# AlerianEmperor/Voxel-Cone-Tracing

Hardware: AMD Instinct MI355X
Metric: Mcones/s (+ ms per GI pass), Sponza-class 256^3 @1080p (higher is better)
Workload: dtype f32; 1 GPU; procedural atrium (Sponza-class, 257488 tris, seed 1234), 256^3 RGBA8 brick chain, 1920x1080, 6 diffuse + 1 specular cone/px, trace of a resident (GPU-rasterised) G-buffer; voxel_dim=256, width=1920, height=1080, cones_per_pixel=7, bounces=1, anisotropic_mips=False, parallelism=single GPU, trace_variant=0, footprint_records=False, comm_reserved_cus=0, raster_form=direct

## Files before the change

### voxel-cone-tracing_amd/csrc/vct_trace.hip

```cpp
#include <hip/hip_fp16.h>

#include "../../include/vct.h"
#include "vct_internal.h"

typedef int vct_v4i32 __attribute__((ext_vector_type(4)));
typedef float vct_v4f32 __attribute__((ext_vector_type(4)));
__device__ vct_v4f32 vct_struct_buffer_load_format_v4f32(vct_v4i32 rsrc, int vindex, int voffset, int soffset, int aux)
    __asm("llvm.amdgcn.struct.buffer.load.format.v4f32");

namespace {

struct F3 { float x, y, z; };
struct F4 { float x, y, z, w; };

__device__ __forceinline__ F3 f3(float x, float y, float z) { return {x, y, z}; }
__device__ __forceinline__ float dot3(F3 a, F3 b) { return a.x * b.x + a.y * b.y + a.z * b.z; }
__device__ __forceinline__ F3 cross3(F3 a, F3 b) {
    return {a.y * b.z - a.z * b.y, a.z * b.x - a.x * b.z, a.x * b.y - a.y * b.x};
}
__device__ __forceinline__ float div_rn(float a, float b) { return a / b; }
__device__ __forceinline__ float sqrt_rn(float a) { return __builtin_sqrtf(a); }
__device__ __forceinline__ F3 normalize3(F3 a) {
    const float l = sqrt_rn(dot3(a, a));
    return {div_rn(a.x, l), div_rn(a.y, l), div_rn(a.z, l)};
// ... 100 lines not shown
        ay = __builtin_amdgcn_readlane(j0, src) - 1;
        az = __builtin_amdgcn_readlane(k0, src) - 1;
        dx = i0 - ax; dy = j0 - ay; dz = k0 - az;
        const uint32_t far = max(max((uint32_t)dx, (uint32_t)dy), (uint32_t)dz);
        const unsigned long long out = ballot64(far > 2u) & am;
        coop = out == 0ull;
    }
    if (COOP && coop) {
        uint32_t idx;
        if (WRAP) {
            const uint32_t m4 = (uint32_t)m << 2;
            const uint32_t sax = spread_byte(lb.lut, ax, m4) >> 2;
            const uint32_t say = spread_byte(lb.lut, ay, m4) >> 1;
            const uint32_t saz = spread_byte(lb.lut, az, m4);
            idx = (((sax | ~MX) + lb.sbx) & MX) | (((say | ~MY) + lb.sby) & MY) |
                  (((saz | ~MZ) + lb.sbz) & MZ);
        } else {
            const int x = min(max(ax + (lb.lane & 3), 0), m);
            const int y = min(max(ay + ((lb.lane >> 2) & 3), 0), m);
            const int z = min(max(az + (lb.lane >> 4), 0), m);
            idx = vct_morton3((uint32_t)x, (uint32_t)y, (uint32_t)z);
        }
        const float4 d = texel_f32(tb, idx);
        if (PRIO) __builtin_amdgcn_s_setprio(0);
        const bool any_texel = ballot64((__float_as_uint(d.x) | __float_as_uint(d.y) | __float_as_uint(d.z) | __float_as_uint(d.w)) != 0u) != 0ull;
        if (VCT_STATS) { if (any_texel) ++ms.coop_hit; else ++ms.coop_zero; }
        if (any_texel) {
            blk[lb.lane] = d;
            wave_sync();
            const int slot = act ? (dz * 4 + dy) * 4 + dx : 0;
            const float4* q = blk + slot;
            const float a0 = 1.0f - a, b0 = 1.0f - b, c0 = 1.0f - c;
            const float ab00 = a0 * b0, ab10 = a * b0, ab01 = a0 * b, ab11 = a * b;
            {
                const float4 t0 = q[0], t1 = q[1], t2 = q[4], t3 = q[5];
                const float w0 = ab00 * c0, w1 = ab10 * c0, w2 = ab01 * c0, w3 = ab11 * c0;
#define VCT_ACC(ch) r.ch = w0 * t0.ch; r.ch = fmaf(w1, t1.ch, r.ch); r.ch = fmaf(w2, t2.ch, r.ch); r.ch = fmaf(w3, t3.ch, r.ch);
                VCT_ACC(x) VCT_ACC(y) VCT_ACC(z) VCT_ACC(w)
#undef VCT_ACC
            }
            __builtin_amdgcn_sched_barrier(0);
            {
                const float4 t4 = q[16], t5 = q[17], t6 = q[20], t7 = q[21];
                wave_sync();
                const float w4 = ab00 * c, w5 = ab10 * c, w6 = ab01 * c, w7 = ab11 * c;
#define VCT_ACC(ch) r.ch = fmaf(w4, t4.ch, r.ch); r.ch = fmaf(w5, t5.ch, r.ch); r.ch = fmaf(w6, t6.ch, r.ch); r.ch = fmaf(w7, t7.ch, r.ch);
                VCT_ACC(x) VCT_ACC(y) VCT_ACC(z) VCT_ACC(w)
#undef VCT_ACC
            }
        }
    } else {
      if (VCT_STATS) {
          ++ms.fallback; ms.fallback_lanes += (uint32_t)__popcll(am);
          int lo[3] = {act ? i0 : 0x7fffffff, act ? j0 : 0x7fffffff, act ? k0 : 0x7fffffff};
          int hi[3] = {act ? i0 : -0x7fffffff, act ? j0 : -0x7fffffff, act ? k0 : -0x7fffffff};
          for (int off = 32; off > 0; off >>= 1)
              for (int q = 0; q < 3; ++q) { lo[q] = min(lo[q], __shfl_xor(lo[q], off)); hi[q] = max(hi[q], __shfl_xor(hi[q], off)); }
          if (hi[0] - lo[0] <= 2 && hi[1] - lo[1] <= 2 && hi[2] - lo[2] <= 2) ++ms.fallback_fits;
          unsigned long long pending = am;
          int nb = 0;
          while (pending != 0ull && nb < 16) {
              const int src = (int)__ffsll((long long)pending) - 1;
              const int bx = __builtin_amdgcn_readlane(i0, src) - 1, by = __builtin_amdgcn_readlane(j0, src) - 1,
                        bz = __builtin_amdgcn_readlane(k0, src) - 1;
              const bool in = (uint32_t)(i0 - bx) <= 2u && (uint32_t)(j0 - by) <= 2u && (uint32_t)(k0 - bz) <= 2u;
              pending &= ~ballot64(in);
              ++nb;
          }
          int qlo[3] = {act ? i0 : 0x7fffffff, act ? j0 : 0x7fffffff, act ? k0 : 0x7fffffff};
          int qhi[3] = {act ? i0 : -0x7fffffff, act ? j0 : -0x7fffffff, act ? k0 : -0x7fffffff};
          bool qany = act;
          auto widen = [&](int off) {
              for (int q = 0; q < 3; ++q) { qlo[q] = min(qlo[q], __shfl_xor(qlo[q], off)); qhi[q] = max(qhi[q], __shfl_xor(qhi[q], off)); }
              qany = qany || (__shfl_xor((int)qany, off) != 0);
          };
          widen(1); widen(8);
          const int span2 = max(max(qhi[0] - qlo[0], qhi[1] - qlo[1]), qhi[2] - qlo[2]);
          const bool lead2 = (lb.lane & 9) == 0;
          ms.quads_live += (uint32_t)__popcll(ballot64(lead2 && qany));
          ms.quads_fit333 += (uint32_t)__popcll(ballot64(lead2 && qany && span2 <= 1));
          ms.quads_same += (uint32_t)__popcll(ballot64(lead2 && qany && span2 == 0));
          widen(2); widen(16);
          const int span4 = max(max(qhi[0] - qlo[0], qhi[1] - qlo[1]), qhi[2] - qlo[2]);
          const bool lead4 = (lb.lane & 27) == 0;
          ms.quadrants_live += (uint32_t)__popcll(ballot64(lead4 && qany));
          ms.quadrants_fit444 += (uint32_t)__popcll(ballot64(lead4 && qany && span4 <= 2));
          ms.greedy_blocks += (uint32_t)nb;
          if (nb <= 2) ++ms.greedy_le2;
          if (nb <= 3) ++ms.greedy_le3;
          if (nb <= 4) ++ms.greedy_le4;
      }
      if (act) {
        uint32_t mx0, mx1, my0, my1, mz0, mz1;
        if (WRAP) {
            if (!CELLS) {
                const uint32_t m4 = (uint32_t)m << 2;
                const char* lutb = (const char*)lb.lut_vec;
                mx0 = *(const uint32_t*)(lutb + (((uint32_t)i0 << 2) & m4)) >> 2;
                my0 = *(const uint32_t*)(lutb + (((uint32_t)j0 << 2) & m4)) >> 1;
                mz0 = *(const uint32_t*)(lutb + (((uint32_t)k0 << 2) & m4));
            } else {
                mx0 = vct_spread3((uint32_t)i0 & (uint32_t)m);
                my0 = vct_spread3((uint32_t)j0 & (uint32_t)m) << 1;
                mz0 = vct_spread3((uint32_t)k0 & (uint32_t)m) << 2;
            }
            mx1 = ((mx0 | ~MX) + 1u) & MX;
            my1 = ((my0 | ~MY) + 2u) & MY;
            mz1 = ((mz0 | ~MZ) + 4u) & MZ;
        } else {
            const int ci0 = min(max(i0, 0), m), ci1 = min(max(i0 + 1, 0), m);
            const int cj0 = min(max(j0, 0), m), cj1 = min(max(j0 + 1, 0), m);
            const int ck0 = min(max(k0, 0), m), ck1 = min(max(k0 + 1, 0), m);
            mx0 = vct_spread3((uint32_t)ci0); mx1 = vct_spread3((uint32_t)ci1);
            my0 = vct_spread3((uint32_t)cj0) << 1; my1 = vct_spread3((uint32_t)cj1) << 1;
            mz0 = vct_spread3((uint32_t)ck0) << 2; mz1 = vct_spread3((uint32_t)ck1) << 2;
        }
        if (!CELLS) {
            const float a0 = 1.0f - a, b0 = 1.0f - b, c0 = 1.0f - c;
            const float ab00 = a0 * b0, ab10 = a * b0, ab01 = a0 * b, ab11 = a * b;
            {
                const float4 f0 = texel_f32(tb, mx0 | my0 | mz0), f1 = texel_f32(tb, mx1 | my0 | mz0);
                const float w0 = ab00 * c0, w1 = ab10 * c0;
#define VCT_ACC(ch) r.ch = w0 * f0.ch; r.ch = fmaf(w1, f1.ch, r.ch);
                VCT_ACC(x) VCT_ACC(y) VCT_ACC(z) VCT_ACC(w)
#undef VCT_ACC
            }
            __builtin_amdgcn_sched_barrier(0);
            {
                const float4 f2 = texel_f32(tb, mx0 | my1 | mz0), f3 = texel_f32(tb, mx1 | my1 | mz0);
                const float w2 = ab01 * c0, w3 = ab11 * c0;
#define VCT_ACC(ch) r.ch = fmaf(w2, f2.ch, r.ch); r.ch = fmaf(w3, f3.ch, r.ch);
                VCT_ACC(x) VCT_ACC(y) VCT_ACC(z) VCT_ACC(w)
#undef VCT_ACC
            }
            __builtin_amdgcn_sched_barrier(0);
            {
                const float4 f4 = texel_f32(tb, mx0 | my0 | mz1), f5 = texel_f32(tb, mx1 | my0 | mz1);
                const float4 f6 = texel_f32(tb, mx0 | my1 | mz1), f7 = texel_f32(tb, mx1 | my1 | mz1);
                if (PRIO) __builtin_amdgcn_s_setprio(0);
                const float w4 = ab00 * c, w5 = ab10 * c, w6 = ab01 * c, w7 = ab11 * c;
#define VCT_ACC(ch) r.ch = fmaf(w4, f4.ch, r.ch); r.ch = fmaf(w5, f5.ch, r.ch); r.ch = fmaf(w6, f6.ch, r.ch); r.ch = fmaf(w7, f7.ch, r.ch);
                VCT_ACC(x) VCT_ACC(y) VCT_ACC(z) VCT_ACC(w)
#undef VCT_ACC
            }
        } else {
            uint32_t t[8];
            if (WRAP && lv.off != 0u) {
                const char* cb = cells + ((size_t)lv.off << 5);
                const uint32_t ro = (mx0 | my0 | mz0) << 5;
                const uint4 lo = *(const uint4*)(cb + ro);
                const uint4 hi = *(const uint4*)(cb + ro + 16u);
                t[0] = lo.x; t[1] = lo.y; t[2] = lo.z; t[3] = lo.w;
                t[4] = hi.x; t[5] = hi.y; t[6] = hi.z; t[7] = hi.w;
            } else {
                t[0] = base[mx0 | my0 | mz0]; t[1] = base[mx1 | my0 | mz0];
                t[2] = base[mx0 | my1 | mz0]; t[3] = base[mx1 | my1 | mz0];
                t[4] = base[mx0 | my0 | mz1]; t[5] = base[mx1 | my0 | mz1];
                t[6] = base[mx0 | my1 | mz1]; t[7] = base[mx1 | my1 | mz1];
            }
            if (PRIO) __builtin_amdgcn_s_setprio(0);
            const float a0 = 1.0f - a, b0 = 1.0f - b, c0 = 1.0f - c;
            const float wg[8] = {(a0 * b0) * c0, (a * b0) * c0, (a0 * b) * c0, (a * b) * c0,
                                 (a0 * b0) * c,  (a * b0) * c,  (a0 * b) * c,  (a * b) * c};
            r.x = wg[0] * unorm8_of<0, LOOSE>(t[0]);
            r.y = wg[0] * unorm8_of<8, LOOSE>(t[0]);
            r.z = wg[0] * unorm8_of<16, LOOSE>(t[0]);
            r.w = wg[0] * unorm8_of<24, LOOSE>(t[0]);
#pragma unroll
            for (int i = 1; i < 8; ++i) {
                r.x = fmaf(wg[i], unorm8_of<0, LOOSE>(t[i]), r.x);
                r.y = fmaf(wg[i], unorm8_of<8, LOOSE>(t[i]), r.y);
                r.z = fmaf(wg[i], unorm8_of<16, LOOSE>(t[i]), r.z);
                r.w = fmaf(wg[i], unorm8_of<24, LOOSE>(t[i]), r.w);
            }
        }
      }
    }
    return r;
}

struct AnisoCone {
    float wx, wy, wz;
    bool nx, ny, nz;
};

template <bool WRAP, bool COOP>
__device__ __forceinline__ F4 sample_aniso(const VctTraceParams& p, const VctLevelRef lv, float ux,
                                           float uy, float uz, bool act, unsigned long long m,
                                           float4* __restrict__ blk, const LaneBlock& lb, const AnisoCone& ac,
                                           MarchStats& ms) {
    auto chain_of = [&](int d) { return p.aniso + (size_t)d * p.aniso_stride - p.level_off[1]; };
    const unsigned long long mx = ballot64(ac.nx) & m, my = ballot64(ac.ny) & m, mz = ballot64(ac.nz) & m;
    F4 tx, ty, tz;
    bool done = false;
    if (COOP && WRAP) {
        const int mm = lv.m;
        const float fN = lv.fN;
        const float u = fmaf(ux, fN, -0.5f), v = fmaf(uy, fN, -0.5f), w = fmaf(uz, fN, -0.5f);
        const float fu = floorf(u), fv = floorf(v), fw = floorf(w);
        const float a = u - fu, b = v - fv, c = w - fw;
        const int i0 = (int)fu, j0 = (int)fv, k0 = (int)fw;
        const int src = ((m >> 27) & 1ull) ? 27 : (int)__ffsll((long long)m) - 1;
        const int ax = __builtin_amdgcn_readlane(i0, src) - 1;
        const int ay = __builtin_amdgcn_readlane(j0, src) - 1;
        const int az = __builtin_amdgcn_readlane(k0, src) - 1;
        const int dx = i0 - ax, dy = j0 - ay, dz = k0 - az;
        const uint32_t far = max(max((uint32_t)dx, (uint32_t)dy), (uint32_t)dz);
        if ((ballot64(far > 2u) & m) == 0ull) {
            done = true;
            const uint32_t MX = lv.mask_x, MY = MX << 1, MZ = MX << 2;
            const uint32_t m4 = (uint32_t)mm << 2;
            const SpreadLut lut = (SpreadLut)p.spread_lut;
            const uint32_t sax = spread_byte(lut, ax, m4) >> 2;
            const uint32_t say = spread_byte(lut, ay, m4) >> 1;
            const uint32_t saz = spread_byte(lut, az, m4);
            const uint32_t idx = (((sax | ~MX) + lb.sbx) & MX) | (((say | ~MY) + lb.sby) & MY) |
                                 (((saz | ~MZ) + lb.sbz) & MZ);
            const unsigned long long mneg[3] = {mx, my, mz};
            const bool lneg[3] = {ac.nx, ac.ny, ac.nz};
            uint32_t tpos[3], tneg[3];
#pragma unroll
            for (int k = 0; k < 3; ++k) {
                tpos[k] = mneg[k] != m ? (chain_of(2 * k) + lv.off)[idx] : 0u;
                tneg[k] = mneg[k] != 0ull ? (chain_of(2 * k + 1) + lv.off)[idx] : 0u;
            }
            const int slot = act ? (dz * 4 + dy) * 4 + dx : 0;
            const float a0 = 1.0f - a, b0 = 1.0f - b, c0 = 1.0f - c;
            const float ab00 = a0 * b0, ab10 = a * b0, ab01 = a0 * b, ab11 = a * b;
            const float w0 = ab00 * c0, w1 = ab10 * c0, w2 = ab01 * c0, w3 = ab11 * c0;
            const float w4 = ab00 * c, w5 = ab10 * c, w6 = ab01 * c, w7 = ab11 * c;
            float4* alt = p.aniso_alt_slab ? blk + p.aniso_alt_slab : blk;
            F4 out3[3];
#pragma unroll
            for (int k = 0; k < 3; ++k) {
                F4 r = {0.0f, 0.0f, 0.0f, 0.0f};
                if (ballot64((tpos[k] | tneg[k]) != 0u) != 0ull) {
                    auto dec = [](uint32_t t) {
                        float4 d;
                        d.x = unorm8(t & 0xffu); d.y = unorm8((t >> 8) & 0xffu);
                        d.z = unorm8((t >> 16) & 0xffu); d.w = unorm8(t >> 24);
                        return d;
                    };
                    if (mneg[k] != m) blk[lb.lane] = dec(tpos[k]);
                    if (mneg[k] != 0ull) alt[lb.lane] = dec(tneg[k]);
                    wave_sync();
                    const float4* q = (lneg[k] ? alt : blk) + slot;
                    const float4 t0 = q[0], t1 = q[1], t2 = q[4], t3v = q[5];
                    const float4 t4 = q[16], t5 = q[17], t6 = q[20], t7 = q[21];
                    wave_sync();
#define VCT_ACC(ch)                                                                            \
    r.ch = w0 * t0.ch;                                                                         \
    r.ch = fmaf(w1, t1.ch, r.ch); r.ch = fmaf(w2, t2.ch, r.ch); r.ch = fmaf(w3, t3v.ch, r.ch); \
    r.ch = fmaf(w4, t4.ch, r.ch); r.ch = fmaf(w5, t5.ch, r.ch); r.ch = fmaf(w6, t6.ch, r.ch);  \
    r.ch = fmaf(w7, t7.ch, r.ch);
                    VCT_ACC(x) VCT_ACC(y) VCT_ACC(z) VCT_ACC(w)
#undef VCT_ACC
                }
                out3[k] = r;
            }
            tx = out3[0]; ty = out3[1]; tz = out3[2];
        }
    }
    if (!done) {
        auto axis_sample = [&](int axis, bool neg, unsigned long long mn) -> F4 {
            if (mn == 0ull) return sample_level<WRAP, COOP>(chain_of(2 * axis), lv, ux, uy, uz, act, m, blk, lb, ms);
            if (mn == m) return sample_level<WRAP, COOP>(chain_of(2 * axis + 1), lv, ux, uy, uz, act, m, blk, lb, ms);
            const F4 a = sample_level<WRAP, COOP>(chain_of(2 * axis), lv, ux, uy, uz, act && !neg, m & ~mn, blk, lb, ms);
            const F4 b = sample_level<WRAP, COOP>(chain_of(2 * axis + 1), lv, ux, uy, uz, act && neg, mn, blk, lb, ms);
            return neg ? b : a;
        };
        tx = axis_sample(0, ac.nx, mx);
        ty = axis_sample(1, ac.ny, my);
        tz = axis_sample(2, ac.nz, mz);
    }
    F4 r;
    r.x = ac.wx * tx.x; r.x = fmaf(ac.wy, ty.x, r.x); r.x = fmaf(ac.wz, tz.x, r.x);
    r.y = ac.wx * tx.y; r.y = fmaf(ac.wy, ty.y, r.y); r.y = fmaf(ac.wz, tz.y, r.y);
    r.z = ac.wx * tx.z; r.z = fmaf(ac.wy, ty.z, r.z); r.z = fmaf(ac.wz, tz.z, r.z);
    r.w = ac.wx * tx.w; r.w = fmaf(ac.wy, ty.w, r.w); r.w = fmaf(ac.wz, tz.w, r.w);
    return r;
}

typedef const __attribute__((address_space(4))) VctStep* StepTable;

__device__ __forceinline__ VctStep load_step(StepTable t, int k) {
    VctStep s;
    s.dist = t[k].dist; s.occ_rcp = t[k].occ_rcp; s.occ_den = t[k].occ_den; s.frac = t[k].frac;
    s.level = t[k].level; s.level2 = t[k].level2; s.two_levels = t[k].two_levels; s.omf = t[k].omf;
    s.l1.off = t[k].l1.off; s.l1.mask_x = t[k].l1.mask_x; s.l1.fN = t[k].l1.fN; s.l1.m = t[k].l1.m;
    s.l2.off = t[k].l2.off; s.l2.mask_x = t[k].l2.mask_x; s.l2.fN = t[k].l2.fN; s.l2.m = t[k].l2.m;
    return s;
}

#define VCT_MARCH_STEP(st, act, live)                                                                        \
        const float px = start.x + dir.x * st.dist; \
        const float py = start.y + dir.y * st.dist; \
        const float pz = start.z + dir.z * st.dist; \
        const float ux = fmaf(div_const<FASTDIV>(px, p.half_G_aux, p.half_G_rcp), 0.5f, 0.5f); \
        const float uy = fmaf(div_const<FASTDIV>(py, p.half_G_aux, p.half_G_rcp), 0.5f, 0.5f); \
        const float uz = fmaf(div_const<FASTDIV>(pz, p.half_G_aux, p.half_G_rcp), 0.5f, 0.5f); \
        F4 vc = (ANISO && st.level >= 1) ? sample_aniso<WRAP, COOP>(p, st.l1, ux, uy, uz, act, live, blk, lb, ac, ms) \
                                         : sample_level<WRAP, COOP, FASTDIV == 2, CELLS, PRIO>(p.chain, st.l1, ux, uy, uz, act, live, blk, lb, ms, p.cells_biased); \
        if (st.two_levels) { \
            const F4 t2 = ANISO ? sample_aniso<WRAP, COOP>(p, st.l2, ux, uy, uz, act, live, blk + 64, lb, ac, ms) \
                                : sample_level<WRAP, COOP, FASTDIV == 2, CELLS, PRIO>(p.chain, st.l2, ux, uy, uz, act, live, blk + 64, lb, ms, p.cells_biased); \
            const float g = st.omf;       \
            vc.x = fmaf(st.frac, t2.x, g * vc.x); \
            vc.y = fmaf(st.frac, t2.y, g * vc.y); \
            vc.z = fmaf(st.frac, t2.z, g * vc.z); \
            vc.w = fmaf(st.frac, t2.w, g * vc.w); \
        } \
        if (act) { \
            const float oma = 1.0f - alpha; \
            cr = fmaf(oma, vc.x, cr); \
            cg = fmaf(oma, vc.y, cg); \
            cb = fmaf(oma, vc.z, cb); \
            occ = occ + div_const<FASTDIV>(oma * vc.w, st.occ_den, st.occ_rcp); \
            alpha = fmaf(oma, vc.w, alpha); \
            ++steps; \
        }

template <bool WRAP, int FASTDIV, bool COOP, bool ANISO = false, bool CELLS = false, bool PRIO = false>
__device__ __forceinline__ F4 cone_march(const VctTraceParams& p, bool alive, F3 start, F3 dir,
                                         const VctStep* tab_global, int n,
                                         float4* __restrict__ blk, const LaneBlock& lb,
                                         int& steps_out, MarchStats& ms) {
    const StepTable tab = (StepTable)tab_global;
    float cr = 0.0f, cg = 0.0f, cb = 0.0f, alpha = 0.0f, occ = 0.0f;
    int steps = 0;
    AnisoCone ac = {0.0f, 0.0f, 0.0f, false, false, false};
    if (ANISO) {
        ac.wx = dir.x * dir.x; ac.wy = dir.y * dir.y; ac.wz = dir.z * dir.z;
        ac.nx = !(dir.x >= 0.0f); ac.ny = !(dir.y >= 0.0f); ac.nz = !(dir.z >= 0.0f);
    }
    const unsigned long long alive_mask = ballot64(alive);
    if constexpr (!ANISO) {
    auto march_step = [&](const VctStep& st, const bool act, const unsigned long long live) { VCT_MARCH_STEP(st, act, live) };
    VctStep ea = load_step(tab, 0), eb = ea;
    for (int k = 0; k < n;) {
        {
            const bool act = alive && (alpha < p.max_alpha);
            const unsigned long long live = ballot64(alpha < p.max_alpha) & alive_mask;
            if (live == 0ull) break;
            if (VCT_STATS) { ++ms.wave_steps; ms.lane_steps += (uint32_t)__popcll(live); }
            eb = load_step(tab, k + 1 < n ? k + 1 : k);
            march_step(ea, act, live);
            if (++k >= n) break;
        }
        {
            const bool act = alive && (alpha < p.max_alpha);
            const unsigned long long live = ballot64(alpha < p.max_alpha) & alive_mask;
            if (live == 0ull) break;
            if (VCT_STATS) { ++ms.wave_steps; ms.lane_steps += (uint32_t)__popcll(live); }
            ea = load_step(tab, k + 1 < n ? k + 1 : k);
            march_step(eb, act, live);
            ++k;
        }
    }
    } else {
    VctStep nxt = load_step(tab, 0);
    for (int k = 0; k < n; ++k) {
        const bool act = alive && (alpha < p.max_alpha);
        const unsigned long long live = ballot64(alpha < p.max_alpha) & alive_mask;
        if (live == 0ull) break;
        if (VCT_STATS) { ++ms.wave_steps; ms.lane_steps += (uint32_t)__popcll(live); }
        const VctStep st = nxt;
        nxt = load_step(tab, k + 1 < n ? k + 1 : k);
        VCT_MARCH_STEP(st, act, live)
    }
    }
    steps_out = steps;
    return {cr, cg, cb, occ};
}

__device__ __forceinline__ uint32_t pack_half2(float a, float b) {
    const __half ha = __float2half_rn(a), hb = __float2half_rn(b);
    return (uint32_t)__half_as_ushort(ha) | ((uint32_t)__half_as_ushort(hb) << 16);
}

__device__ __forceinline__ void flush_stats(const VctTraceParams& p, const MarchStats& ms, int lane) {
    if (VCT_STATS && p.stats && lane == 0) {
        const uint32_t v[16] = {ms.wave_steps, ms.lane_steps, ms.coop_zero, ms.coop_hit, ms.fallback,
                                ms.fallback_lanes, ms.fallback_fits, ms.greedy_blocks, ms.greedy_le2, ms.greedy_le3,
                                ms.greedy_le4, ms.quads_live, ms.quads_fit333, ms.quads_same, ms.quadrants_live,
                                ms.quadrants_fit444};
        for (int i = 0; i < 16; ++i)
            if (v[i]) atomicAdd(p.stats + i, (unsigned long long)v[i]);
    }
}

__constant__ float kConeDirs[18] = {0.0f, 0.0f, 1.0f,
                                    0.0f, 0.866025f, 0.5f,
                                    0.823639f, 0.267617f, 0.5f,
                                    0.509037f, -0.700629f, 0.5f,
                                    -0.509037f, -0.700629f, 0.5f,
                                    -0.823639f, 0.267617f, 0.5f};
__constant__ float kConeWeights[6] = {0.25f, 0.15f, 0.15f, 0.15f, 0.15f, 0.15f};

__device__ __forceinline__ int xcd_remap(int b, int nblocks) {
    const int run = 16, group = 8 * run;
    const int g = b / group, local = b - g * group;
    return (g + 1) * group <= nblocks ? g * group + (local & 7) * run + (local >> 3) : b;
}

#ifndef VCT_WAVES_PER_BLOCK
#define VCT_WAVES_PER_BLOCK 1
#endif
#ifndef VCT_TRACE_MIN_WAVES
#define VCT_TRACE_MIN_WAVES 7
#endif

template <bool WRAP, int FASTDIV, bool COOP>
__global__ void __launch_bounds__(64 * VCT_WAVES_PER_BLOCK, VCT_TRACE_MIN_WAVES)
k_trace_tile(const VctTraceParams p) {
    __shared__ float4 lds_blk[VCT_WAVES_PER_BLOCK][2][64];
    const int lane = threadIdx.x & 63;
    const int wave = __builtin_amdgcn_readfirstlane((int)(threadIdx.x >> 6));
    float4* blk = &lds_blk[wave][0][0];
    LaneBlock lb;

    const int ntiles = (p.tile_row1 - p.tile_row0) * p.tiles_x;
    const int vb = xcd_remap((int)blockIdx.x, (int)gridDim.x);
    const int ti = vb * VCT_WAVES_PER_BLOCK + wave;
    if (ti >= ntiles) return;

    lb.lane = lane;
    lb.lut = (SpreadLut)p.spread_lut; lb.lut_vec = p.spread_lut;
    lb.sbx = vct_spread3((uint32_t)lane & 3u);     
    lb.sby = vct_spread3(((uint32_t)lane >> 2) & 3u) << 1;
    lb.sbz = vct_spread3((uint32_t)lane >> 4) << 2;
    MarchStats ms = {};

    const int tile = p.tile_row0 * p.tiles_x + ti;
    const int ty = tile / p.tiles_x, tx = tile - ty * p.tiles_x;
    auto fresh_lane = [&]() { int l = lane; asm volatile("" : "+v"(l)); return l; };
    auto pixel_index = [&](int l) {
        return (size_t)(ty * VCT_TILE + (l >> 3)) * p.width + (tx * VCT_TILE + (l & 7));
    };
    auto gbuf_ptr = [&](int l) {
        return p.gbuf + (size_t)tile * (VCT_GB_NPLANES * VCT_TILE_PIX) + l;
    };
    const int x = tx * VCT_TILE + (lane & 7), y = ty * VCT_TILE + (lane >> 3);
    const float* gb = gbuf_ptr(lane);
#define VCT_GB(k) gb[(k) * VCT_TILE_PIX]
    const bool in_frame = (x < p.width) && (y < p.height);
    const bool alive = in_frame && !(VCT_GB(18) < 0.5f);

    F3 start, k0, k1, k2;
    {
        const F3 P = f3(VCT_GB(0), VCT_GB(1), VCT_GB(2)), Nw = f3(VCT_GB(3), VCT_GB(4), VCT_GB(5));
        const F3 T = f3(VCT_GB(6), VCT_GB(7), VCT_GB(8)), B = f3(VCT_GB(9), VCT_GB(10), VCT_GB(11));
        const F3 c0 = cross3(B, Nw), c1 = cross3(Nw, T), c2 = cross3(T, B);
        const float inv_det = div_rn(1.0f, dot3(T, c0));
        k0 = f3(c0.x * inv_det, c0.y * inv_det, c0.z * inv_det);
        k1 = f3(c1.x * inv_det, c1.y * inv_det, c1.z * inv_det);
        k2 = f3(c2.x * inv_det, c2.y * inv_det, c2.z * inv_det);
        start = f3(P.x + Nw.x * p.vs, P.y + Nw.y * p.vs, P.z + Nw.z * p.vs);
    }

    float ind[4] = {0.0f, 0.0f, 0.0f, 0.0f};
    int total = 0;
#pragma unroll 1
    for (int i = 0; i < 6; ++i) {
        const float ddx = kConeDirs[3 * i], ddy = kConeDirs[3 * i + 1], ddz = kConeDirs[3 * i + 2];
        F3 dir = f3(k0.x * ddx + k1.x * ddy + k2.x * ddz, k0.y * ddx + k1.y * ddy + k2.y * ddz,
                    k0.z * ddx + k1.z * ddy + k2.z * ddz);
        dir = normalize3(dir);
        int st;
        const F4 c = cone_march<WRAP, FASTDIV, COOP>(p, alive, start, dir, p.steps_diffuse,
                                                     p.n_diffuse, blk, lb, st, ms);
        total += st;
        const float wgt = kConeWeights[i];
        ind[0] = fmaf(wgt, c.x, ind[0]);
        ind[1] = fmaf(wgt, c.y, ind[1]);
        ind[2] = fmaf(wgt, c.z, ind[2]);
        ind[3] = fmaf(wgt, c.w, ind[3]);
        if (p.dbg_cones && alive) {
            float* d = p.dbg_cones + pixel_index(fresh_lane()) * 28 + 4 * i;
            d[0] = c.x; d[1] = c.y; d[2] = c.z; d[3] = c.w;
        }
        if (p.dbg_steps && in_frame) p.dbg_steps[pixel_index(fresh_lane()) * 7 + i] = (uint8_t)st;
    }

    const float* gb2 = gbuf_ptr(fresh_lane());
#undef VCT_GB
#define VCT_GB(k) gb2[(k) * VCT_TILE_PIX]
    F4 sc;
    {
        const F3 P = f3(VCT_GB(0), VCT_GB(1), VCT_GB(2));
        const F3 N = f3(VCT_GB(12), VCT_GB(13), VCT_GB(14));
        const F3 E = normalize3(f3(p.cam[0] - P.x, p.cam[1] - P.y, p.cam[2] - P.z));
        const F3 Rd = normalize3(reflect3(f3(E.x * -1.0f, E.y * -1.0f, E.z * -1.0f), N));
        int st6;
        sc = cone_march<WRAP, FASTDIV, COOP>(p, alive, start, Rd, p.steps_specular, p.n_specular,
                                             blk, lb, st6, ms);
        total += st6;
        if (p.dbg_cones && alive) {
            float* d = p.dbg_cones + pixel_index(fresh_lane()) * 28 + 24;
            d[0] = sc.x; d[1] = sc.y; d[2] = sc.z; d[3] = sc.w;
        }
        if (p.dbg_steps && in_frame) p.dbg_steps[pixel_index(fresh_lane()) * 7 + 6] = (uint8_t)st6;
    }

    const float* gb3 = gbuf_ptr(fresh_lane());
#undef VCT_GB
#define VCT_GB(k) gb3[(k) * VCT_TILE_PIX]
    if (in_frame) {
        const F3 P = f3(VCT_GB(0), VCT_GB(1), VCT_GB(2));
        const F3 N = f3(VCT_GB(12), VCT_GB(13), VCT_GB(14));
        const float alb_r = VCT_GB(15), alb_g = VCT_GB(16), alb_b = VCT_GB(17), alb_a = VCT_GB(18);
        const float shadow = VCT_GB(22);
        const F3 L = normalize3(f3(p.light[0], p.light[1], p.light[2]));
        const F3 E = normalize3(f3(p.cam[0] - P.x, p.cam[1] - P.y, p.cam[2] - P.z));
        const float cos_theta = fmaxf(dot3(N, L), 0.0f);
        const float direct_diffuse = shadow * cos_theta;
        const float occlusion = 1.0f - ind[3];
        const float dr = (direct_diffuse + occlusion * ind[0]) * alb_r;
        const float dg = (direct_diffuse + occlusion * ind[1]) * alb_g;
        const float db = (direct_diffuse + occlusion * ind[2]) * alb_b;
        const F3 R = normalize3(reflect3(f3(L.x * -1.0f, L.y * -1.0f, L.z * -1.0f), N));
        const float spec = powf(fmaxf(dot3(E, R), 0.0f), p.shininess);
        const float direct_spec = spec * shadow;
        const float spec_occ = 1.0f - sc.w;
        const float sr = (sc.x + spec_occ * direct_spec) * VCT_GB(19);
        const float sg = (sc.y + spec_occ * direct_spec) * VCT_GB(20);
        const float sb = (sc.z + spec_occ * direct_spec) * VCT_GB(21);
        const float ar = p.ambient * alb_r * occlusion;
        const float ag = p.ambient * alb_g * occlusion;
        const float ab = p.ambient * alb_b * occlusion;
        float o0 = ar + dr + sr, o1 = ag + dg + sg, o2 = ab + db + sb, o3 = alb_a;
        if (!alive) {
            const float cc = p.ambient < 0.5f ? 0.5f : 1.0f;
            o0 = cc; o1 = cc; o2 = cc; o3 = 1.0f;
        }
        uint2 pk;
        pk.x = pack_half2(o0, o1);
        pk.y = pack_half2(o2, o3);
        *reinterpret_cast<uint2*>(p.out + pixel_index(fresh_lane()) * 4) = pk;
    }
#undef VCT_GB
    for (int off = 32; off > 0; off >>= 1) total += __shfl_xor(total, off);
    if (lane == 0) p.tile_steps[tile] = (uint32_t)total;
    flush_stats(p, ms, lane);
}

#ifndef VCT_SPLIT
#define VCT_SPLIT 3
#endif
#define VCT_CONES_PER_WAVE (6 / (VCT_SPLIT - 1))
static_assert(VCT_SPLIT == 3 || VCT_SPLIT == 4 || VCT_SPLIT == 7, "VCT_SPLIT must be 3, 4 or 7");
#ifndef VCT_ANISO_MIN_WAVES
#define VCT_ANISO_MIN_WAVES 5
#endif

template <bool WRAP, int FASTDIV, bool ANISO, bool COMPACT = false, bool CELLS = false, bool PRIO = false, bool COMP = false>
__global__ void __launch_bounds__(64 * VCT_SPLIT, ANISO ? VCT_ANISO_MIN_WAVES : VCT_TRACE_MIN_WAVES)
k_trace_tile_split(const VctTraceParams p) {
    __shared__ float4 lds_blk[VCT_SPLIT][ANISO ? 4 : 2][64];
    __shared__ float4 lds_cone[7][64];
    __shared__ int lds_done;
    __shared__ int lds_steps;
    const int lane = threadIdx.x & 63;
    const int wave = __builtin_amdgcn_readfirstlane((int)(threadIdx.x >> 6));
    float4* blk = &lds_blk[wave][0][0];
    LaneBlock lb;
    if (threadIdx.x == 0) { lds_done = 0; lds_steps = 0; }
    __syncthreads();

    const int ntiles = p.ntiles;
    const int ti = xcd_remap((int)blockIdx.x, (int)gridDim.x);
    if (ti >= ntiles) return;
    constexpr bool compact = COMPACT;
    uint32_t cpix = 0u;
    if (compact) {
        if ((uint32_t)ti >= *p.vt_count) {
            if (threadIdx.x == 0) p.tile_steps[p.tile_row0 * p.tiles_x + ti] = 0u;
            return;
        }
        cpix = p.vt_pix[(size_t)ti * 64 + lane];
    }

    lb.lane = lane;
    lb.lut = (SpreadLut)p.spread_lut; lb.lut_vec = p.spread_lut;
    lb.sbx = vct_spread3((uint32_t)lane & 3u);     
    lb.sby = vct_spread3(((uint32_t)lane >> 2) & 3u) << 1;
    lb.sbz = vct_spread3((uint32_t)lane >> 4) << 2;
    MarchStats ms = {};

    int lrow = 0, tile0 = p.tile_row0 * p.tiles_x + ti;
    if (p.row_stride > 1) {
        lrow = ti / p.tiles_x;
        tile0 = (p.tile_row0 + lrow * p.row_stride) * p.tiles_x + (ti - lrow * p.tiles_x);
    }
    const bool cvalid = !compact || cpix != 0xffffffffu;
    const int tile = compact ? (cvalid ? (int)(cpix >> 6) : 0) : tile0;
    const int ty = tile / p.tiles_x, tx = tile - ty * p.tiles_x;
    const int oy = p.pack_rows ? (p.row_stride > 1 ? lrow : ty - p.tile_row0) : ty;
    const int plane_ = compact ? (int)(cpix & 63u) : lane;
    auto fresh_lane = [&]() { int l = plane_; asm volatile("" : "+v"(l)); return l; };
    auto pixel_index = [&](int l) {
        return (size_t)(oy * VCT_TILE + (l >> 3)) * p.width + (tx * VCT_TILE + (l & 7));
    };
    auto gbuf_ptr = [&](int l) {
        return p.gbuf + (size_t)tile * (VCT_GB_NPLANES * VCT_TILE_PIX) + l;
    };
    const int x = tx * VCT_TILE + (plane_ & 7), y = ty * VCT_TILE + (plane_ >> 3);
    const float* gb = gbuf_ptr(plane_);
#define VCT_GB(k) gb[(k) * VCT_TILE_PIX]
    const bool in_frame = cvalid && (x < p.width) && (y < p.height);
    const bool alive = in_frame && !(VCT_GB(18) < 0.5f);
    int total = 0;
    const uint32_t groups = COMP ? (uint32_t)__builtin_amdgcn_readfirstlane((int)p.comp) >> VCT_COMP_GROUPS_SHIFT : 3u;
    const int n_diffuse = (groups & 1u) ? p.n_diffuse : 0, n_specular = (groups & 2u) ? p.n_specular : 0;
    if (wave < VCT_SPLIT - 1) {
        F3 start, k0, k1, k2;
        {
            const F3 P = f3(VCT_GB(0), VCT_GB(1), VCT_GB(2)), Nw = f3(VCT_GB(3), VCT_GB(4), VCT_GB(5));
            const F3 T = f3(VCT_GB(6), VCT_GB(7), VCT_GB(8)), B = f3(VCT_GB(9), VCT_GB(10), VCT_GB(11));
            const F3 c0 = cross3(B, Nw), c1 = cross3(Nw, T), c2 = cross3(T, B);
            const float inv_det = div_rn(1.0f, dot3(T, c0));
            k0 = f3(c0.x * inv_det, c0.y * inv_det, c0.z * inv_det);
            k1 = f3(c1.x * inv_det, c1.y * inv_det, c1.z * inv_det);
            k2 = f3(c2.x * inv_det, c2.y * inv_det, c2.z * inv_det);
            start = f3(P.x + Nw.x * p.vs, P.y + Nw.y * p.vs, P.z + Nw.z * p.vs);
        }
#pragma unroll 1
        for (int i = wave * VCT_CONES_PER_WAVE; i < wave * VCT_CONES_PER_WAVE + VCT_CONES_PER_WAVE; ++i) {
            const float ddx = kConeDirs[3 * i], ddy = kConeDirs[3 * i + 1], ddz = kConeDirs[3 * i + 2];
            F3 dir = f3(k0.x * ddx + k1.x * ddy + k2.x * ddz, k0.y * ddx + k1.y * ddy + k2.y * ddz,
                        k0.z * ddx + k1.z * ddy + k2.z * ddz);
            dir = normalize3(dir);
            int st;
            const F4 c = cone_march<WRAP, FASTDIV, true, ANISO, CELLS, PRIO>(p, alive, start, dir, p.steps_diffuse,
                                                                n_diffuse, blk, lb, st, ms);
            total += st;
            lds_cone[i][lane] = make_float4(c.x, c.y, c.z, c.w);
            if (p.dbg_cones && alive) {
                float* d = p.dbg_cones + pixel_index(fresh_lane()) * 28 + 4 * i;
                d[0] = c.x; d[1] = c.y; d[2] = c.z; d[3] = c.w;
            }
            if (p.dbg_steps && in_frame) p.dbg_steps[pixel_index(fresh_lane()) * 7 + i] = (uint8_t)st;
        }
    } else {
        if (!PRIO && p.spec_prio) __builtin_amdgcn_s_setprio(1);
        const F3 P = f3(VCT_GB(0), VCT_GB(1), VCT_GB(2)), Nw = f3(VCT_GB(3), VCT_GB(4), VCT_GB(5));
        const F3 N = f3(VCT_GB(12), VCT_GB(13), VCT_GB(14));
        const F3 start = f3(P.x + Nw.x * p.vs, P.y + Nw.y * p.vs, P.z + Nw.z * p.vs);
        const F3 E = normalize3(f3(p.cam[0] - P.x, p.cam[1] - P.y, p.cam[2] - P.z));
        const F3 Rd = normalize3(reflect3(f3(E.x * -1.0f, E.y * -1.0f, E.z * -1.0f), N));
        int st6;
        const F4 sc = cone_march<WRAP, FASTDIV, true, ANISO, CELLS, PRIO>(p, alive, start, Rd, p.steps_specular,
                                                             n_specular, blk, lb, st6, ms);
        total += st6;
        lds_cone[6][lane] = make_float4(sc.x, sc.y, sc.z, sc.w);
        if (p.dbg_cones && alive) {
            float* d = p.dbg_cones + pixel_index(fresh_lane()) * 28 + 24;
            d[0] = sc.x; d[1] = sc.y; d[2] = sc.z; d[3] = sc.w;
        }
        if (p.dbg_steps && in_frame) p.dbg_steps[pixel_index(fresh_lane()) * 7 + 6] = (uint8_t)st6;
    }
    for (int off = 32; off > 0; off >>= 1) total += __shfl_xor(total, off);
    if (lane == 0) atomicAdd(&lds_steps, total);
    flush_stats(p, ms, lane);

    __threadfence_block();
    int arrived = 0;
    if (lane == 0) arrived = atomicAdd(&lds_done, 1);
    arrived = __builtin_amdgcn_readfirstlane(arrived);
    if (arrived != VCT_SPLIT - 1) return;
    __threadfence_block();
    if (lane == 0) p.tile_steps[tile0] = (uint32_t)lds_steps;

    const float* gb3 = gbuf_ptr(fresh_lane());
#undef VCT_GB
#define VCT_GB(k) gb3[(k) * VCT_TILE_PIX]
    if (in_frame) {
        float ind[4] = {0.0f, 0.0f, 0.0f, 0.0f};
#pragma unroll
        for (int i = 0; i < 6; ++i) {
            const float4 c = lds_cone[i][lane];
            const float wgt = kConeWeights[i];
            ind[0] = fmaf(wgt, c.x, ind[0]);
            ind[1] = fmaf(wgt, c.y, ind[1]);
            ind[2] = fmaf(wgt, c.z, ind[2]);
            ind[3] = fmaf(wgt, c.w, ind[3]);
        }
        const float4 sc = lds_cone[6][lane];
        const F3 P = f3(VCT_GB(0), VCT_GB(1), VCT_GB(2));
        const F3 N = f3(VCT_GB(12), VCT_GB(13), VCT_GB(14));
        const float alb_r = VCT_GB(15), alb_g = VCT_GB(16), alb_b = VCT_GB(17), alb_a = VCT_GB(18);
        const float shadow = VCT_GB(22);
        const F3 L = normalize3(f3(p.light[0], p.light[1], p.light[2]));
        const F3 E = normalize3(f3(p.cam[0] - P.x, p.cam[1] - P.y, p.cam[2] - P.z));
        const float cos_theta = fmaxf(dot3(N, L), 0.0f);
        const uint32_t comp = COMP ? (uint32_t)__builtin_amdgcn_readfirstlane((int)p.comp) : 0u;
        const uint32_t show = COMP ? comp & (uint32_t)VCT_SHOW_ALL : (uint32_t)VCT_SHOW_ALL;
        const bool s_dd = !COMP || (show & VCT_SHOW_DIFFUSE), s_ao = !COMP || (show & VCT_SHOW_AMBIENT_OCCLUSION);
        const bool s_ird = !COMP || (show & VCT_SHOW_INDIRECT_DIFFUSE), s_ds = !COMP || (show & VCT_SHOW_SPECULAR);
        const bool s_irs = !COMP || (show & VCT_SHOW_INDIRECT_SPECULAR);
        const float raw_dd = shadow * cos_theta;
        const float direct_diffuse = s_dd ? raw_dd : 0.0f;
        const float occlusion = s_ao ? 1.0f - ind[3] : 1.0f;
        const float ird_r = s_ird ? ind[0] : 0.0f, ird_g = s_ird ? ind[1] : 0.0f, ird_b = s_ird ? ind[2] : 0.0f;
        const float dr = (direct_diffuse + occlusion * ird_r) * alb_r;
        const float dg = (direct_diffuse + occlusion * ird_g) * alb_g;
        const float db = (direct_diffuse + occlusion * ird_b) * alb_b;
        const F3 R = normalize3(reflect3(f3(L.x * -1.0f, L.y * -1.0f, L.z * -1.0f), N));
        const float spec = powf(fmaxf(dot3(E, R), 0.0f), p.shininess);
        const float raw_ds = spec * shadow;
        const float direct_spec = s_ds ? raw_ds : 0.0f;
        const float spec_occ = s_ao ? 1.0f - sc.w : 1.0f;
        const float irs_r = s_irs ? sc.x : 0.0f, irs_g = s_irs ? sc.y : 0.0f, irs_b = s_irs ? sc.z : 0.0f;
        const float sr = (irs_r + spec_occ * direct_spec) * VCT_GB(19);
        const float sg = (irs_g + spec_occ * direct_spec) * VCT_GB(20);
        const float sb = (irs_b + spec_occ * direct_spec) * VCT_GB(21);
        const float ar = p.ambient * alb_r * occlusion;
        const float ag = p.ambient * alb_g * occlusion;
        const float ab = p.ambient * alb_b * occlusion;
        float o0 = ar + dr + sr, o1 = ag + dg + sg, o2 = ab + db + sb, o3 = alb_a;
        if (!alive) {
            const float cc = p.ambient < 0.5f ? 0.5f : 1.0f;
            o0 = cc; o1 = cc; o2 = cc; o3 = 1.0f;
        }
        uint2 pk;
        pk.x = pack_half2(o0, o1);
        pk.y = pack_half2(o2, o3);
        *reinterpret_cast<uint2*>(p.out + pixel_index(fresh_lane()) * 4) = pk;
        if (COMP) {
            const uint32_t which = comp >> VCT_COMP_AOV_SHIFT;
            const size_t frame_halves = (size_t)p.width * p.height * 4;
            uint16_t* dst = p.aov + pixel_index(fresh_lane()) * 4;
            uint2 q;
            if (which & VCT_AOV_INDIRECT_DIFFUSE) {
                q.x = alive ? pack_half2(ind[0], ind[1]) : 0u;
                q.y = alive ? pack_half2(ind[2], ind[3]) : 0u;
                *reinterpret_cast<uint2*>(dst) = q;
                dst += frame_halves;
            }
            if (which & VCT_AOV_INDIRECT_SPECULAR) {
                q.x = alive ? pack_half2(sc.x, sc.y) : 0u;
                q.y = alive ? pack_half2(sc.z, sc.w) : 0u;
                *reinterpret_cast<uint2*>(dst) = q;
                dst += frame_halves;
            }
            if (which & VCT_AOV_DIRECT) {
                q.x = alive ? pack_half2(raw_dd, raw_ds) : 0u;
                q.y = alive ? pack_half2(shadow, 1.0f) : 0u;
                *reinterpret_cast<uint2*>(dst) = q;
            }
        }
    }
#undef VCT_GB
}

__device__ __forceinline__ uint32_t to_unorm8_dev(float f) {
    const float s = f * 255.0f + 0.5f;
    if (!(s > 0.0f)) return 0u;
    if (s >= 255.0f) return 255u;
    return (uint32_t)(int)s;
}

template <class March>
__device__ __forceinline__ void bounce_voxels(const VctTraceParams& p, bool alive, size_t vox, int& total_out,
                                              March march) {
    const uint32_t* __restrict__ level0 = p.chain;
    const float fV = (float)p.V;
    const uint32_t slot = p.brick_slot[vox >> 9];
    const size_t pv = (size_t)(slot == VCT_NO_SLOT ? 0u : slot) * 512 + (vox & 511u);
    const uint32_t src = level0[vox], nq = p.attr_normal[pv], aq = p.attr_albedo[pv];
    const uint32_t mi = (uint32_t)vox;
    const int i = (int)vct_compact3(mi), j = (int)vct_compact3(mi >> 1), k = (int)vct_compact3(mi >> 2);
    const F3 P = f3((div_rn((float)i + 0.5f, fV) - 0.5f) * p.G, (div_rn((float)j + 0.5f, fV) - 0.5f) * p.G,
                    (div_rn((float)k + 0.5f, fV) - 0.5f) * p.G);
    const F3 nrm = normalize3(f3((float)((int)(nq & 0xffu) - 128), (float)((int)((nq >> 8) & 0xffu) - 128),
                                 (float)((int)((nq >> 16) & 0xffu) - 128)));
    const F3 helper = fabsf(nrm.y) < 0.9f ? f3(0.0f, 1.0f, 0.0f) : f3(1.0f, 0.0f, 0.0f);
    const F3 t = normalize3(cross3(helper, nrm));
    const F3 bt = cross3(nrm, t);
    const F3 start = f3(P.x + nrm.x * p.vs, P.y + nrm.y * p.vs, P.z + nrm.z * p.vs);
    float ind[4] = {0.0f, 0.0f, 0.0f, 0.0f};
    int total = 0;
#pragma unroll 1
    for (int c = 0; c < 6; ++c) {
        const float ddx = kConeDirs[3 * c], ddy = kConeDirs[3 * c + 1], ddz = kConeDirs[3 * c + 2];
        F3 dir = f3(t.x * ddx + bt.x * ddy + nrm.x * ddz, t.y * ddx + bt.y * ddy + nrm.y * ddz,
                    t.z * ddx + bt.z * ddy + nrm.z * ddz);
        dir = normalize3(dir);
        int st;
        const F4 cone = march(alive, start, dir, st);
        total += st;
        const float wgt = kConeWeights[c];
        ind[0] = fmaf(wgt, cone.x, ind[0]);
        ind[1] = fmaf(wgt, cone.y, ind[1]);
        ind[2] = fmaf(wgt, cone.z, ind[2]);
        ind[3] = fmaf(wgt, cone.w, ind[3]);
    }
    if (alive) {
        const float occlusion = 1.0f - ind[3];
        const uint32_t r = to_unorm8_dev(unorm8(src & 0xffu) + unorm8(aq & 0xffu) * (occlusion * ind[0]));
        const uint32_t g = to_unorm8_dev(unorm8((src >> 8) & 0xffu) + unorm8((aq >> 8) & 0xffu) * (occlusion * ind[1]));
        const uint32_t bl = to_unorm8_dev(unorm8((src >> 16) & 0xffu) + unorm8((aq >> 16) & 0xffu) * (occlusion * ind[2]));
        p.bounce_out[vox] = r | (g << 8) | (bl << 16) | (src & 0xff000000u);
    } else {
        total = 0;
    }
    for (int off = 32; off > 0; off >>= 1) total += __shfl_xor(total, off);
    total_out = total;
}

#define VCT_BOUNCE_SETUP                                                     \
    __shared__ float4 lds_blk[VCT_WAVES_PER_BLOCK][2][64];                   \
    const int lane = threadIdx.x & 63;                                       \
    const int wave = __builtin_amdgcn_readfirstlane((int)(threadIdx.x >> 6)); \
    float4* blk = &lds_blk[wave][0][0];                                      \
    LaneBlock lb;                                                            \
    lb.lane = lane;                                                          \
    lb.lut = (SpreadLut)p.spread_lut; lb.lut_vec = p.spread_lut;                                        \
    lb.sbx = vct_spread3((uint32_t)lane & 3u);                               \
    lb.sby = vct_spread3(((uint32_t)lane >> 2) & 3u) << 1;                   \
    lb.sbz = vct_spread3((uint32_t)lane >> 4) << 2;                          \
    MarchStats ms = {};

__device__ __forceinline__ int compact_brick(const VctTraceParams& p, uint32_t b, int lane, uint16_t* list) {
    const uint32_t slot = p.brick_slot[b];
    const bool has = slot != VCT_NO_SLOT;
    const uint32_t* __restrict__ src = p.chain + (size_t)b * 512 + lane;
    const uint32_t* __restrict__ nrm = p.attr_normal + (size_t)(has ? slot : 0u) * 512 + lane;
    uint32_t t[8], a[8];
#pragma unroll
    for (int it = 0; it < 8; ++it) { t[it] = src[it * 64]; a[it] = nrm[it * 64]; }
    int n = 0;
#pragma unroll
    for (int it = 0; it < 8; ++it) {
        p.bounce_out[(size_t)b * 512 + it * 64 + lane] = t[it];
        const bool occ = (t[it] >> 24) != 0u && has && (a[it] & 0xffffffu) != 0x808080u;
        const unsigned long long m = ballot64(occ);
        if (occ) list[n + __popcll(m & ((1ull << lane) - 1ull))] = (uint16_t)(it * 64 + lane);
        n += __popcll(m);
    }
    return n;
}

#define VCT_BLIST_WAVES 16
__global__ void __launch_bounds__(64 * VCT_BLIST_WAVES)
k_bounce_list(const VctTraceParams p) {
    __shared__ uint16_t lds_list[VCT_BLIST_WAVES][512];
    __shared__ uint32_t lds_n[VCT_BLIST_WAVES];
    __shared__ uint32_t lds_base;
    const int lane = threadIdx.x & 63;
    const int wave = __builtin_amdgcn_readfirstlane((int)(threadIdx.x >> 6));
    uint16_t* list = &lds_list[wave][0];
    const uint32_t nwaves = gridDim.x * VCT_BLIST_WAVES;
    const uint32_t nchunks = (p.nbricks + 63u) >> 6;
    for (uint32_t c = blockIdx.x * VCT_BLIST_WAVES + wave; c < nchunks; c += nwaves) {
        const uint32_t mine = c * 64u + (uint32_t)lane;
        const bool stale = mine < p.nbricks && p.brick_prev[mine] == 0u && p.bounce_seen[mine] != 0u;
        for (unsigned long long m = ballot64(stale); m != 0ull; m &= m - 1ull) {
            const uint32_t b = c * 64u + (uint32_t)(__ffsll((long long)m) - 1);
            for (int it = 0; it < 8; ++it) p.bounce_out[(size_t)b * 512 + it * 64 + lane] = 0u;
        }
    }
    for (uint32_t s0 = blockIdx.x * VCT_BLIST_WAVES; s0 < p.nslots; s0 += nwaves) {
        const uint32_t sl = s0 + (uint32_t)wave;
        uint32_t b = 0u;
        int n = 0;
        if (sl < p.nslots) {
            b = p.slot_brick[sl];
            if (p.brick_prev[b]) n = compact_brick(p, b, lane, list);
        }
        if (lane == 0) lds_n[wave] = (uint32_t)n;
        __syncthreads();
        if (threadIdx.x == 0) {
            uint32_t total = 0u;
            for (int w = 0; w < VCT_BLIST_WAVES; ++w) total += lds_n[w];
            lds_base = total ? atomicAdd(p.bounce_list_count, total) : 0u;
        }
        __syncthreads();
        if (n != 0) {
            uint32_t off = lds_base;
            for (int w = 0; w < wave; ++w) off += lds_n[w];
            if (off + (uint32_t)n > p.bounce_list_cap) {
                if (lane == 0) p.brick_over[b] = 1u;
                for (uint32_t i = off + (uint32_t)lane; i < p.bounce_list_cap; i += 64u) p.bounce_list[i] = 0xffffffffu;
            } else {
                for (int i = lane; i < n; i += 64) p.bounce_list[off + i] = b * 512u + list[i];
            }
        }
        __syncthreads();
    }
}

#ifndef VCT_BOUNCE_MIN_WAVES
#define VCT_BOUNCE_MIN_WAVES 5
#endif
template <bool WRAP, int FASTDIV>
__global__ void __launch_bounds__(64 * VCT_WAVES_PER_BLOCK, VCT_BOUNCE_MIN_WAVES)
k_bounce_march(const VctTraceParams p) {
    VCT_BOUNCE_SETUP
    const uint32_t n = min(*p.bounce_list_count, p.bounce_list_cap);
    const uint32_t nwaves = gridDim.x * VCT_WAVES_PER_BLOCK;
    unsigned long long wave_steps = 0;
    for (uint32_t w = blockIdx.x * VCT_WAVES_PER_BLOCK + wave; w * 64u < n; w += nwaves) {
        const uint32_t e = w * 64u + lane < n ? p.bounce_list[w * 64u + lane] : 0xffffffffu;
        const bool alive = e != 0xffffffffu;
        const uint32_t first = __builtin_amdgcn_readfirstlane(e);
        const size_t vox = alive ? e : (first != 0xffffffffu ? first : 0u);
        int total;
        bounce_voxels(p, alive, vox, total, [&](bool al, F3 start, F3 dir, int& st) {
            return cone_march<WRAP, FASTDIV, true>(p, al, start, dir, p.steps_diffuse, p.n_diffuse, blk, lb, st, ms);
        });
        wave_steps += (unsigned long long)total;
    }
    if (lane == 0 && wave_steps)
        atomicAdd(p.step_counter + ((blockIdx.x * VCT_WAVES_PER_BLOCK + wave) & (VCT_STEP_COUNTERS - 1)), wave_steps);
}

template <bool WRAP, int FASTDIV>
__global__ void __launch_bounds__(64 * VCT_WAVES_PER_BLOCK, VCT_BOUNCE_MIN_WAVES)
k_bounce_bricks(const VctTraceParams p) {
    VCT_BOUNCE_SETUP
    __shared__ uint16_t lds_list[VCT_WAVES_PER_BLOCK][512];
    uint16_t* list = &lds_list[wave][0];
    unsigned long long wave_steps = 0;
    const uint32_t nwaves = gridDim.x * VCT_WAVES_PER_BLOCK;
    const uint32_t nchunks = (p.nslots + 63u) >> 6;
    for (uint32_t c = blockIdx.x * VCT_WAVES_PER_BLOCK + wave; c < nchunks; c += nwaves) {
        const uint32_t sl = c * 64u + (uint32_t)lane;
        const uint32_t mine = sl < p.nslots ? p.slot_brick[sl] : 0u;
        const bool over = sl < p.nslots && p.brick_over[mine] != 0u;
        if (over) p.brick_over[mine] = 0u;
        for (unsigned long long m = ballot64(over); m != 0ull; m &= m - 1ull) {
            const uint32_t b = (uint32_t)__builtin_amdgcn_readlane((int)mine, __ffsll((long long)m) - 1);
            const int n = compact_brick(p, b, lane, list);
            wave_sync();
            for (int base = 0; base < n; base += 64) {
                const bool alive = base + lane < n;
                const size_t vox = (size_t)b * 512 + (alive ? list[base + lane] : list[base]);
                int total;
                bounce_voxels(p, alive, vox, total, [&](bool al, F3 start, F3 dir, int& st) {
                    return cone_march<WRAP, FASTDIV, true>(p, al, start, dir, p.steps_diffuse, p.n_diffuse, blk, lb, st, ms);
                });
                wave_steps += (unsigned long long)total;
            }
            wave_sync();
        }
    }
    if (lane == 0 && wave_steps)
        atomicAdd(p.step_counter + ((blockIdx.x * VCT_WAVES_PER_BLOCK + wave) & (VCT_STEP_COUNTERS - 1)), wave_steps);
}

__global__ void __launch_bounds__(256)
k_compact_tiles(const VctTraceParams p) {
    const int lane = threadIdx.x & 63;
    const int rows = p.tile_row1 - p.tile_row0;
    const int sx_n = (p.tiles_x + 1) >> 1, sy_n = (rows + 1) >> 1;
    const int st = blockIdx.x * (blockDim.x >> 6) + (int)(threadIdx.x >> 6);
    if (st >= sx_n * sy_n) return;
    const int sy = st / sx_n, sx = st - sy * sx_n;
    unsigned long long m[4];
    int tiles[4];
#pragma unroll
    for (int k = 0; k < 4; ++k) {
        const int tx = 2 * sx + (k & 1), ty = p.tile_row0 + 2 * sy + (k >> 1);
        const bool have = tx < p.tiles_x && ty < p.tile_row1;
        tiles[k] = have ? ty * p.tiles_x + tx : -1;
        bool live = false;
        if (have) {
            const int x = tx * VCT_TILE + (lane & 7), y = ty * VCT_TILE + (lane >> 3);
            const bool in_frame = x < p.width && y < p.height;
            const float a = p.gbuf[(size_t)tiles[k] * (VCT_GB_NPLANES * VCT_TILE_PIX) + 18 * VCT_TILE_PIX + lane];
            live = in_frame && !(a < 0.5f);
            if (in_frame && !live) {
                const float cc = p.ambient < 0.5f ? 0.5f : 1.0f;
                uint2 pk;
                pk.x = pack_half2(cc, cc);
                pk.y = pack_half2(cc, 1.0f);
                *reinterpret_cast<uint2*>(p.out + ((size_t)y * p.width + x) * 4) = pk;
            }
        }
        m[k] = ballot64(live);
    }
    const int total = (int)(__popcll(m[0]) + __popcll(m[1]) + __popcll(m[2]) + __popcll(m[3]));
    const int nvt = (total + 63) >> 6;
    uint32_t base = 0u;
    if (lane == 0 && nvt) base = atomicAdd(p.vt_count, (uint32_t)nvt);
    base = (uint32_t)__builtin_amdgcn_readfirstlane((int)base);
    int n = 0;
#pragma unroll
    for (int k = 0; k < 4; ++k) {
        if ((m[k] >> lane) & 1ull)
// ... 133 lines not shown
```

Baseline: 26910 Mcones/s.

## Shrink trace kernel LDS footprint by sharing one sample slab and packing cone results

For the isotropic, non-CELLS, 3-wave split kernel, each wave now uses a single LDS sample slab instead of two, and both mip-level samples share it. Cone results are packed into fewer LDS slots: wave 0 accumulates its weighted diffuse cones in place, and the other waves store into a reduced lds_cone array or reuse their own sample slab. This cuts per-block LDS from about 17KB to roughly 6KB, which may allow more resident blocks per CU. The risk is that reusing one slab for both levels could serialise the two samples or create a hazard if they overlap in time, and the final-combine reads now depend on the slab reuse being correct.

```diff
diff --git a/voxel-cone-tracing_amd/csrc/vct_trace.hip b/voxel-cone-tracing_amd/csrc/vct_trace.hip
--- a/voxel-cone-tracing_amd/csrc/vct_trace.hip
+++ b/voxel-cone-tracing_amd/csrc/vct_trace.hip
@@ -426,8 +426,9 @@
         F4 vc = (ANISO && st.level >= 1) ? sample_aniso<WRAP, COOP>(p, st.l1, ux, uy, uz, act, live, blk, lb, ac, ms) \
                                          : sample_level<WRAP, COOP, FASTDIV == 2, CELLS, PRIO>(p.chain, st.l1, ux, uy, uz, act, live, blk, lb, ms, p.cells_biased); \
         if (st.two_levels) { \
+             \
             const F4 t2 = ANISO ? sample_aniso<WRAP, COOP>(p, st.l2, ux, uy, uz, act, live, blk + 64, lb, ac, ms) \
-                                : sample_level<WRAP, COOP, FASTDIV == 2, CELLS, PRIO>(p.chain, st.l2, ux, uy, uz, act, live, blk + 64, lb, ms, p.cells_biased); \
+                                : sample_level<WRAP, COOP, FASTDIV == 2, CELLS, PRIO>(p.chain, st.l2, ux, uy, uz, act, live, ONE_SLAB ? blk : blk + 64, lb, ms, p.cells_biased); \
             const float g = st.omf;       \
             vc.x = fmaf(st.frac, t2.x, g * vc.x); \
             vc.y = fmaf(st.frac, t2.y, g * vc.y); \
@@ -444,7 +445,7 @@
             ++steps; \
         }
 
-template <bool WRAP, int FASTDIV, bool COOP, bool ANISO = false, bool CELLS = false, bool PRIO = false>
+template <bool WRAP, int FASTDIV, bool COOP, bool ANISO = false, bool CELLS = false, bool PRIO = false, bool ONE_SLAB = false>
 __device__ __forceinline__ F4 cone_march(const VctTraceParams& p, bool alive, F3 start, F3 dir,
                                          const VctStep* tab_global, int n,
                                          float4* __restrict__ blk, const LaneBlock& lb,
@@ -680,8 +681,9 @@
 template <bool WRAP, int FASTDIV, bool ANISO, bool COMPACT = false, bool CELLS = false, bool PRIO = false, bool COMP = false>
 __global__ void __launch_bounds__(64 * VCT_SPLIT, ANISO ? VCT_ANISO_MIN_WAVES : VCT_TRACE_MIN_WAVES)
 k_trace_tile_split(const VctTraceParams p) {
-    __shared__ float4 lds_blk[VCT_SPLIT][ANISO ? 4 : 2][64];
-    __shared__ float4 lds_cone[7][64];
+    constexpr bool SMALL_LDS = !ANISO && !CELLS && VCT_SPLIT == 3;
+    __shared__ float4 lds_blk[VCT_SPLIT][ANISO ? 4 : SMALL_LDS ? 1 : 2][64];
+    __shared__ float4 lds_cone[SMALL_LDS ? 3 : 7][64];
     __shared__ int lds_done;
     __shared__ int lds_steps;
     const int lane = threadIdx.x & 63;
@@ -755,10 +757,23 @@
                         k0.z * ddx + k1.z * ddy + k2.z * ddz);
             dir = normalize3(dir);
             int st;
-            const F4 c = cone_march<WRAP, FASTDIV, true, ANISO, CELLS, PRIO>(p, alive, start, dir, p.steps_diffuse,
+            const F4 c = cone_march<WRAP, FASTDIV, true, ANISO, CELLS, PRIO, SMALL_LDS>(p, alive, start, dir, p.steps_diffuse,
                                                                 n_diffuse, blk, lb, st, ms);
             total += st;
-            lds_cone[i][lane] = make_float4(c.x, c.y, c.z, c.w);
+            if (!SMALL_LDS) {
+                lds_cone[i][lane] = make_float4(c.x, c.y, c.z, c.w);
+            } else if (wave == 0) {
+                const float wgt = kConeWeights[i];
+                float4 ind = i == 0 ? make_float4(0.0f, 0.0f, 0.0f, 0.0f) : lds_cone[2][lane];
+                ind.x = fmaf(wgt, c.x, ind.x);
+                ind.y = fmaf(wgt, c.y, ind.y);
+                ind.z = fmaf(wgt, c.z, ind.z);
+                ind.w = fmaf(wgt, c.w, ind.w);
+                lds_cone[2][lane] = ind;
+            } else {
+                float4* dst = i < 5 ? &lds_cone[i - 3][0] : blk;
+                dst[lane] = make_float4(c.x, c.y, c.z, c.w);
+            }
             if (p.dbg_cones && alive) {
                 float* d = p.dbg_cones + pixel_index(fresh_lane()) * 28 + 4 * i;
                 d[0] = c.x; d[1] = c.y; d[2] = c.z; d[3] = c.w;
@@ -773,10 +788,10 @@
         const F3 E = normalize3(f3(p.cam[0] - P.x, p.cam[1] - P.y, p.cam[2] - P.z));
         const F3 Rd = normalize3(reflect3(f3(E.x * -1.0f, E.y * -1.0f, E.z * -1.0f), N));
         int st6;
-        const F4 sc = cone_march<WRAP, FASTDIV, true, ANISO, CELLS, PRIO>(p, alive, start, Rd, p.steps_specular,
+        const F4 sc = cone_march<WRAP, FASTDIV, true, ANISO, CELLS, PRIO, SMALL_LDS>(p, alive, start, Rd, p.steps_specular,
                                                              n_specular, blk, lb, st6, ms);
         total += st6;
-        lds_cone[6][lane] = make_float4(sc.x, sc.y, sc.z, sc.w);
+        (SMALL_LDS ? blk : &lds_cone[6][0])[lane] = make_float4(sc.x, sc.y, sc.z, sc.w);
         if (p.dbg_cones && alive) {
             float* d = p.dbg_cones + pixel_index(fresh_lane()) * 28 + 24;
             d[0] = sc.x; d[1] = sc.y; d[2] = sc.z; d[3] = sc.w;
@@ -800,16 +815,20 @@
 #define VCT_GB(k) gb3[(k) * VCT_TILE_PIX]
     if (in_frame) {
         float ind[4] = {0.0f, 0.0f, 0.0f, 0.0f};
+        if (SMALL_LDS) {
+            const float4 i0 = lds_cone[2][lane];
+            ind[0] = i0.x; ind[1] = i0.y; ind[2] = i0.z; ind[3] = i0.w;
+        }
 #pragma unroll
-        for (int i = 0; i < 6; ++i) {
-            const float4 c = lds_cone[i][lane];
+        for (int i = SMALL_LDS ? 3 : 0; i < 6; ++i) {
+            const float4 c = SMALL_LDS ? (i < 5 ? lds_cone[i - 3][lane] : lds_blk[1][0][lane]) : lds_cone[i][lane];
             const float wgt = kConeWeights[i];
             ind[0] = fmaf(wgt, c.x, ind[0]);
             ind[1] = fmaf(wgt, c.y, ind[1]);
             ind[2] = fmaf(wgt, c.z, ind[2]);
             ind[3] = fmaf(wgt, c.w, ind[3]);
         }
-        const float4 sc = lds_cone[6][lane];
+        const float4 sc = SMALL_LDS ? lds_blk[2][0][lane] : lds_cone[6][lane];
         const F3 P = f3(VCT_GB(0), VCT_GB(1), VCT_GB(2));
         const F3 N = f3(VCT_GB(12), VCT_GB(13), VCT_GB(14));
         const float alb_r = VCT_GB(15), alb_g = VCT_GB(16), alb_b = VCT_GB(17), alb_a = VCT_GB(18);
```

Result: no change. 26960 Mcones/s, median of 6 (+0.2%).
